# michalfratczak/habdec

Hardware: AMD Instinct MI355X
Metric: IQ Msamples/s (batched 2.048 MS/s streams) (higher is better)
Workload: dtype f32

## Files before the change

### habdec_amd/capi.py

```python
from __future__ import annotations

import ctypes as C
from pathlib import Path

import numpy as np

LIB_PATH = Path(__file__).resolve().parent / "libhabdec_amd.so"
_lib = None


class HabdecError(RuntimeError):
    pass


class hd_engine_config(C.Structure):
    _fields_ = [("device", C.c_int32), ("n_streams", C.c_uint32), ("max_chunk", C.c_uint32), ("sampling_rate", C.c_double),
                ("decimation", C.c_uint32), ("baud", C.c_double), ("rtty_bits", C.c_uint32), ("rtty_stops", C.c_float),
                ("lowpass_bw_hz", C.c_float), ("lowpass_trans", C.c_float), ("dc_remove", C.c_int32), ("lookup_mode", C.c_int32),
                ("enable_spectrum", C.c_int32), ("ungated", C.c_int32), ("keep_filtered", C.c_int32), ("pipeline", C.c_int32), ("arith", C.c_int32)]


class hd_afc_info(C.Structure):
    _fields_ = [("frequency_correction", C.c_double), ("shift_hz", C.c_double), ("noise_floor", C.c_double),
                ("noise_variance", C.c_double), ("peak_left", C.c_int32), ("peak_right", C.c_int32), ("spectra", C.c_uint64)]


class hd_timing(C.Structure):
    _fields_ = [("ms_total", C.c_double), ("ms_front", C.c_double), ("front_bytes", C.c_uint64), ("samples", C.c_uint64),
                ("host_enqueue_us", C.c_double), ("host_wait_us", C.c_double), ("host_text_us", C.c_double), ("timed_calls", C.c_uint64),
                ("path", C.c_uint32), ("step_variant", C.c_uint32), ("host_calls_in_place", C.c_uint64), ("lowpass_fft_calls", C.c_uint64)]


class hd_tune_info(C.Structure):
    _fields_ = [("offset_hz", C.c_double), ("step", C.c_uint32), ("phase", C.c_uint32), ("retunes", C.c_uint64), ("from_call", C.c_uint64),
                ("auto_afc", C.c_int32)]


class hd_front_tune_info(C.Structure):
    _fields_ = [("offset_hz", C.c_double), ("step", C.c_uint32), ("phase", C.c_uint32), ("from_call", C.c_uint64)]


SENTENCE_CB = C.CFUNCTYPE(None, C.c_void_p, C.c_uint32, C.c_char_p, C.c_char_p, C.c_char_p)
MATCH_CB = C.CFUNCTYPE(None, C.c_void_p, C.c_uint32, C.c_char_p, C.c_char_p, C.c_char_p, C.c_int)
CHARS_CB = C.CFUNCTYPE(None, C.c_void_p, C.c_uint32, C.POINTER(C.c_char), C.c_size_t)

# ... 27 lines not shown
    "hd_set_match_callback": (None, [_vp, MATCH_CB, _vp]),
    "hd_set_chars_callback": (None, [_vp, CHARS_CB, _vp]),
    "hd_process_host": (_int, [_vp, _vp, _sz, _vp, _u32]),
    "hd_process_device": (_int, [_vp, _vp, _sz, _vp, _u32]),
    "hd_flush": (_int, [_vp]),
    "hd_ingest_run": (_int, [_vp, _vp, C.c_uint64, C.POINTER(C.c_uint64)]),
    "hd_stream_rtty": (_sz, [_vp, _u32, C.c_char_p, _sz]),
    "hd_stream_last_sentence": (_sz, [_vp, _u32, C.c_char_p, _sz]),
    "hd_stream_take_sentences": (_sz, [_vp, _u32, C.c_char_p, _sz]),
    "hd_stream_take_matches": (_sz, [_vp, _u32, C.c_char_p, _sz]),
    "hd_stream_take_chars": (_sz, [_vp, _u32, C.c_char_p, _sz]),
    "hd_engine_sentences_ok": (C.c_uint64, [_vp]),
    "hd_stream_afc": (_int, [_vp, _u32, C.POINTER(hd_afc_info)]),
    "hd_stream_spectrum": (_sz, [_vp, _u32, _f32p, _sz]),
    "hd_stream_power": (_sz, [_vp, _u32, _f32p, _sz]),
    "hd_stream_demodulated": (_sz, [_vp, _u32, _f32p, _sz]),
    "hd_stream_decimated": (_sz, [_vp, _u32, _f32p, _sz]),
    "hd_stream_filtered": (_sz, [_vp, _u32, _f32p, _sz]),
    "hd_stream_bits": (_sz, [_vp, _u32, _u8p, _sz]),
    "hd_stream_flips": (_sz, [_vp, _u32, _u32p, _sz]),
    "hd_stream_fir_taps": (_sz, [_vp, _u32, _f32p, _sz]),
    "hd_stream_symbol_backlog": (_u32, [_vp, _u32]),
    "hd_stream_bits_total": (C.c_uint64, [_vp, _u32]),
    "hd_stream_flip_list_full": (C.c_uint64, [_vp, _u32]),
    "hd_stream_demod_checksum": (C.c_int, [_vp, _u32, C.POINTER(C.c_uint64), C.POINTER(C.c_uint32), C.POINTER(C.c_uint32)]),
    "hd_stream_demod_checksum_total": (C.c_int, [_vp, _u32, C.POINTER(C.c_uint64), C.POINTER(C.c_uint64), C.POINTER(C.c_uint64)]),
    "hd_min_chunk": (_u32, [_u32]),
    "hd_engine_timing": (_int, [_vp, C.POINTER(hd_timing)]),
    "hd_engine_set_timing": (None, [_vp, _int]),
}
# ... 67 lines not shown
```

### habdec_amd/csrc/dev_types.h

```cpp
#pragma once
#include <stdint.h>
#ifndef __HIPCC__
#ifndef __host__
#define __host__
#define __device__
#endif
#endif

namespace hd {

constexpr int kFftBins = 4096;
constexpr uint32_t kVentLimit = 30000;
constexpr uint32_t kFirBatch = 256;

struct StreamCall {
    uint32_t n_in;
    uint32_t n1;
    uint32_t n2;
    uint32_t zero_hist1;
    uint32_t zero_hist2;
    uint32_t pend_before;
    uint32_t fft_fill;
    uint32_t fft_take;
    uint32_t fft_run;
    uint32_t fir_m;
    uint32_t fir_taps;
    uint32_t fir_zero_hist;
    uint32_t pend_after;
    uint32_t dc_remove;
    uint32_t clear_pending;
    uint32_t fir_taps_prev;
};
__host__ __device__ inline uint32_t sc_taps_prev(const StreamCall& c) { return c.fir_taps_prev & 0xFFFFu; }
__host__ __device__ inline uint32_t sc_head_n(const StreamCall& c) { return (c.fir_taps_prev >> 16) & 0x3FFFu; }
__host__ __device__ inline bool sc_head_prev(const StreamCall& c) { return (c.fir_taps_prev >> 30) & 1u; }
__host__ __device__ inline bool sc_head_save(const StreamCall& c) { return (c.fir_taps_prev >> 31) & 1u; }
__host__ __device__ inline uint32_t sc_pack_taps_prev(uint32_t taps_prev, uint32_t head_n, bool head_prev, bool head_save)
{ return (taps_prev & 0xFFFFu) | ((head_n & 0x3FFFu) << 16) | ((head_prev ? 1u : 0u) << 30) | ((head_save ? 1u : 0u) << 31); }


struct SymbolParams {
    uint32_t spb;
    uint32_t R;
    uint32_t min_held;
    uint32_t float_abs;
    uint32_t reset;
};
// ... 33 lines not shown
```

### habdec_amd/csrc/engine.cpp

```cpp
#include <hip/hip_runtime.h>
#include <rocfft/rocfft.h>

#include <algorithm>
#include <atomic>
#include <chrono>
#include <cmath>
#include <cstdio>
#include <cstdlib>
#include <cstring>
#include <memory>
#include <condition_variable>
#include <mutex>
#include <thread>
#include <string>
#include <vector>

#include "../../include/habdec_amd.h"
#include "dev_types.h"
#include "host/afc_tracker.hpp"
#include "host/decim_plan.hpp"
#include "host/fir_design.hpp"
#include "host/iq_file_batch.hpp"
#include "host/text_stage.hpp"
#include "host/tune_host.hpp"
// ... 33 lines not shown
    hipError_t alloc(size_t count)
    {
        n = count;
        hipError_t e = hipHostMalloc(reinterpret_cast<void**>(&p), std::max<size_t>(count, 1) * sizeof(T), hipHostMallocMapped | hipHostMallocCoherent);
        if (e == hipSuccess) std::memset(p, 0, std::max<size_t>(count, 1) * sizeof(T));
        if (e == hipSuccess) e = hipHostGetDevicePointer(reinterpret_cast<void**>(&dev), p, 0);
        return e;
    }
    ~PinBuf() { if (p) (void)hipHostFree(p); }
};

struct SizeState {
    size_t stage_buf[2] = {0, 0};
    size_t pending = 0;
    size_t fft_fill = 0;
    size_t fir_buf = 0;
    uint32_t fir_T_run = 0;
    uint32_t head_n = 0;
    uint64_t head_call = ~0ull;
    bool head_aside = false;
    uint32_t tune_phase = 0;
    uint32_t front_phase = 0;
    uint32_t win_ub = 0, inflight_m = 0;
    uint32_t last_n2 = 0, last_pend_before = 0, last_m = 0;
    int last_buf = 0;
};

struct StreamHost {
    double baud = 300;
    float lp_bw = 1500, lp_trans = 0.025f;
    bool dc = false;
    hd::LowpassDesigner lp;
    bool taps_dirty = false;
    uint32_t tune_step = 0;
    uint32_t held = 0;
    bool sym_reset = true;
    hd::TextStage text;
    hd::AfcTracker afc;
    hd::SpectrumStats stats{};
    bool have_spectrum = false;
    uint64_t spectra = 0;
    uint32_t last_nbits = 0, last_nflips = 0;
    uint64_t flip_list_full = 0;
    uint64_t bits_total = 0;
    std::vector<uint32_t> last_words;
    uint32_t demod_ck[2] = {0, 0}, demod_ck_n = 0xFFFFFFFFu;
    uint64_t demod_ck_call = 0;
    uint64_t demod_ck_hash = 0xCBF29CE484222325ull;
    uint64_t demod_ck_calls = 0, demod_ck_unknown = 0;
    double tune_hz = 0;
    uint64_t tune_from = 0, retunes = 0;
    bool auto_afc = false;
    double afc_hold_s = 6.0, afc_min_hz = 100.0;
    uint64_t afc_elapsed = 0;
    double front_hz = 0;
// ... 9 lines not shown
    std::vector<hd::DecimStage> stages;
    uint32_t S = 0, D = 1;
    uint32_t n1_cap = 0, n2_cap = 0;
    uint32_t taps_cap = 0, fir_hist_cap = 0;
    size_t fbuf_stride = 0;
    uint32_t tail_cap = 0, backlog_cap = 0, slot_words = 0, flips_cap = 0, max_R = 0, min_R = 4;
    int bins_sep = 8;
    bool decode_enabled = true;
    bool fast = false;
    bool one_stream = false;
    bool no_tail = false;
    uint32_t tail_max_n2 = 2048;
    int last_route = -1;
    struct PendingTail { bool valid = false; hd::TailArgs ta{}; int slot = 0; int r2 = 0, t2 = 0; } pend;
    DevBuf<float2> fft_tw;
    bool no_claim = false;
    uint32_t step_run = 0;
    bool no_cu_step = false;
    uint32_t ring_run = 0;
    uint32_t ring_short_pct = 25;
    static constexpr uint32_t kS1Loaders = 2;
#ifndef HD_S1_SLOTS_BATCH
#define HD_S1_SLOTS_BATCH 4
#endif
    static constexpr uint32_t kS1Slots = HD_S1_SLOTS_BATCH;
    PinBuf<unsigned int> ring_gave_up;
    std::string fail_cause;
    bool device_failed = false;
    uint64_t step_launches = 0;
    DevBuf<unsigned int> step_ctr;
// ... 35 lines not shown
    DevBuf<uint32_t> demod_ck_acc;
    uint32_t head_cap = 0;
    DevBuf<hd::SymbolParams> d_sym;
    PinBuf<hd::SymbolParams> h_sym;
    static constexpr int kSlots = 4;
    struct CallSlot {
        DevBuf<hd::StreamCall> d_call;
        PinBuf<hd::StreamCall> h_call;
        PinBuf<uint32_t> h_slots;
        PinBuf<hd::SpectrumStatsDev> h_stats;
        PinBuf<uint2> h_tune;
        PinBuf<uint2> h_front;
        bool timed = false, timed_step = false;
        hipEvent_t ev_front = nullptr, ev_done = nullptr, ev_params = nullptr, ev_spec = nullptr, t0 = nullptr, t1 = nullptr, t2 = nullptr, t3 = nullptr;
        bool busy = false;
        uint32_t seq = 0;
        uint64_t total_in = 0;
        uint32_t r1 = 1;
        ~CallSlot() { for (hipEvent_t ev : {ev_front, ev_done, ev_params, ev_spec, t0, t1, t2, t3}) if (ev) (void)hipEventDestroy(ev); }
    } slot[kSlots];
    uint64_t calls = 0;
    uint64_t delivered = 0;
    int cur = 0;
    int hist_cur = 0;
    int carry_cur = 0;
    bool sym_dirty = true;

    std::vector<StreamHost> st;
    std::vector<SizeState> mirror, mirror_next;
    std::recursive_mutex mtx;
// ... 205 lines not shown
    HD_HIP(e->h_sym.alloc(S));
    for (auto& sl : e->slot) {
        HD_HIP(sl.d_call.alloc(S));
        HD_HIP(sl.h_call.alloc(S));
        HD_HIP(sl.h_slots.alloc((size_t)S * e->slot_words));
        HD_HIP(sl.h_tune.alloc(S));
        HD_HIP(sl.h_front.alloc(S));
    }
    {
        std::vector<float> tab(4 * hd::kTuneTable);
        hd::tune_tables(tab.data(), tab.data() + 2 * hd::kTuneTable);
        HD_HIP(e->tune_tab.alloc(tab.size()));
        HD_HIP(hipMemcpy(e->tune_tab.p, tab.data(), tab.size() * sizeof(float), hipMemcpyHostToDevice));
    }
    if (cfg->enable_spectrum) {
        HD_HIP(e->fft_in.alloc((size_t)S * hd::kFftBins));
        HD_HIP(e->spec.alloc((size_t)S * hd::kFftBins));
        HD_HIP(e->power.alloc((size_t)S * hd::kFftBins));
        for (auto& sl : e->slot) HD_HIP(sl.h_stats.alloc(S));
        {
            std::vector<float2> tw(hd::kFftBins);
            for (size_t m = 0; m < hd::kFftBins; ++m) {
                const double a = 2.0 * 3.14159265358979323846264338327950288 * (double)m / (double)hd::kFftBins;
                tw[m] = make_float2((float)std::cos(a), (float)-std::sin(a));
            }
            HD_HIP(e->fft_tw.alloc(hd::kFftBins));
            HD_HIP(hipMemcpy(e->fft_tw.p, tw.data(), tw.size() * sizeof(float2), hipMemcpyHostToDevice));
        }
    }
    if (e->fast && e->taps_cap >= hd_engine::kLpFftMinTaps && getenv("HD_NO_LP_FFT") == nullptr) {
        std::call_once(g_rocfft_once, [] { rocfft_setup(); });
// ... 65 lines not shown
    (void)hipDeviceSynchronize();
    delete e;
}

uint32_t hd_engine_streams(const hd_engine* e) { return e ? e->S : 0; }
uint32_t hd_engine_decimation(const hd_engine* e) { return e ? e->D : 0; }
double hd_engine_decimated_rate(const hd_engine* e) { return e ? e->fsd : 0; }
uint64_t hd_engine_sentences_ok(const hd_engine* e) { return e ? e->sentences_ok : 0; }
void hd_engine_set_timing(hd_engine* e, int on) { if (e) e->timing_every = on < 0 ? 0u : (uint32_t)on; }
int hd_engine_timing(hd_engine* e, hd_timing* out)
{
    if (!e || !out) return fail(HD_ERR_INVALID, "null argument");
    *out = e->last_timing;
    out->host_calls_in_place = e->host_calls_in_place;
    out->lowpass_fft_calls = e->lpf_calls;
    return HD_OK;
}

extern "C" int hd_debug_step_counters(hd_engine* e, unsigned int* out32)
{
    if (!e || !out32) return HD_ERR_INVALID;
    std::vector<unsigned int> h(2 * 16 * 32);
    if (hipDeviceSynchronize() != hipSuccess || hipMemcpy(h.data(), e->step_ctr.p, h.size() * 4, hipMemcpyDeviceToHost) != hipSuccess) return HD_ERR_DEVICE;
    for (int i = 0; i < 32; ++i) out32[i] = h[(size_t)i * 32];
    return HD_OK;
}

void hd_set_sentence_callback(hd_engine* e, hd_sentence_cb cb, void* user) { if (e) { e->sentence_cb = cb; e->sentence_user = user; } }
void hd_set_match_callback(hd_engine* e, hd_match_cb cb, void* user) { if (e) { e->match_cb = cb; e->match_user = user; } }
void hd_set_chars_callback(hd_engine* e, hd_chars_cb cb, void* user) { if (e) { e->chars_cb = cb; e->chars_user = user; } }
// ... 179 lines not shown
    }
    if (e->device_failed && rc == HD_OK)
        rc = fail(HD_ERR_DEVICE, e->fail_cause + ": the results of this and of every later call of this engine are unreliable -- destroy the engine");
    if (e->device_failed) {
        e->last_timing.host_wait_us = std::chrono::duration<double, std::micro>(w1 - w0).count();
        e->last_timing.host_text_us = 0;
        return rc;
    }
    for (uint32_t s = 0; s < e->S; ++s) {
        StreamHost& st = e->st[s];
        const hd::StreamCall& c = sl.h_call.p[s];
        if (c.fft_run) {
            std::memcpy(&st.stats, &sl.h_stats.p[s], sizeof(st.stats));
            st.have_spectrum = true;
            ++st.spectra;
        }
        const bool past_batch_gate = c.fir_m || c.clear_pending;
        if (past_batch_gate && e->cfg.enable_spectrum) st.afc.step(st.have_spectrum, st.stats, hd::kFftBins, e->fsd);
        st.afc_elapsed += c.n_in;
        if (st.auto_afc && (double)st.afc_elapsed >= st.afc_hold_s * e->fs && std::abs(st.afc.correction) > st.afc_min_hz) {
            const double corr = st.afc.correction;
            uint32_t d = 0;
            if (hd::tune_step(st.tune_hz + corr, e->fsd, &d)) {
                st.tune_hz += corr; st.tune_step = d; st.tune_from = e->calls;
                if (!d) e->mirror[s].tune_phase = 0;
                st.afc.reset(corr, hd::kFftBins, e->fsd);
                st.afc_elapsed = 0;
                ++st.retunes;
            }
        }
// ... 100 lines not shown
        const uint32_t n = n_per_stream ? n_per_stream[s] : n_uniform;
        c.n_in = n;
        c.n1 = n / p.R1;
        c.n2 = c.n1 / p.R2;
        if (n) {
            if (p.nst > 0) { const size_t want = (size_t)n + p.T1 + p.R1; if (nx.stage_buf[0] < want) { nx.stage_buf[0] = want; c.zero_hist1 = 1; } }
            if (p.nst > 1) { const size_t want = (size_t)c.n1 + p.T2 + p.R2; if (nx.stage_buf[1] < want) { nx.stage_buf[1] = want; c.zero_hist2 = 1; } }
        }
        c.dc_remove = st.dc && c.n2;
        sl.h_tune.p[s] = make_uint2(st.tune_step, nx.tune_phase);
        if (st.tune_step) { p.any_tune = true; nx.tune_phase += c.n2 * st.tune_step; }
        sl.h_front.p[s] = make_uint2(st.front_step, nx.front_phase);
        if (st.front_step | nx.front_phase) { p.any_front = true; nx.front_phase += n * st.front_step; }
        c.pend_before = (uint32_t)nx.pending;
        nx.pending += c.n2;
        c.fft_fill = (uint32_t)nx.fft_fill;
        if (e->cfg.enable_spectrum && n && nx.fft_fill < (size_t)hd::kFftBins && c.n2) {
            c.fft_take = (uint32_t)std::min<size_t>(hd::kFftBins - nx.fft_fill, c.n2);
            nx.fft_fill += c.fft_take;
        }
        if (e->cfg.enable_spectrum && n && nx.fft_fill >= (size_t)hd::kFftBins) { c.fft_run = 1; nx.fft_fill = 0; p.any_fft = true; }
        const bool past_batch_gate = n && nx.pending >= hd::kFirBatch;
        nx.last_m = 0;
        if (past_batch_gate && !e->decode_enabled) { c.clear_pending = 1; nx.pending = 0; }
        else if (past_batch_gate) {
            const uint32_t m = (uint32_t)(nx.pending - nx.pending % hd::kFirBatch);
            st.lp.batch = m;
            if (st.lp.design(cutoff_rel(e, st), st.lp_trans)) {
                st.taps_dirty = true;
                redesigned = true;
            }
            const uint32_t T = (uint32_t)st.lp.taps.size();
            if (!T) return fail(HD_ERR_UNSUPPORTED, "low-pass transition width leaves no taps (reference filters nothing then)");
            if (T > e->taps_cap) return fail(HD_ERR_CAPACITY, "low-pass tap count exceeds engine capacity");
            if (nx.fir_buf < (size_t)m + T) { nx.fir_buf = (size_t)m + T; c.fir_zero_hist = 1; }
            c.fir_m = m; c.fir_taps = T;
// ... 38 lines not shown
    r = CallRoute{};
    r.tail_lanes = S >= 2 * e->n_cus ? 64 : 256;
    const bool tail = p.nst == 2 && !p.any_dc && !e->no_tail && p.max_n2 <= e->tail_max_n2 &&
                      ((r.tail_lanes == 256 && p.max_n2 >= 512u && HDK(tail_layout, r.ta, r.tail_lanes, R2, T2, p.max_taps, e->max_R, e->min_R, e->tail_cap, p.max_pend, 64 * 1024, 4)) ||
                       HDK(tail_layout, r.ta, r.tail_lanes, R2, T2, p.max_taps, e->max_R, e->min_R, e->tail_cap, p.max_pend, 64 * 1024));
    const uint32_t step_lds = (p.R1 == 32 || p.R1 == 64) ? HDK(step_lds_bytes, (int)p.R1, (int)p.T1) : 0u;
    const bool step = tail && !p.any_front && e->cfg.pipeline && !e->one_stream && p.min_in == p.max_in && p.max_in && step_lds &&
                      HDK(tail_layout, r.ta_step, 64, R2, T2, p.max_taps, e->max_R, e->min_R, e->tail_cap, p.max_pend, step_lds);
    r.route = step ? Route::step : tail ? Route::tail : Route::separate;
    r.any_post = p.any_dc || (p.any_tune && !tail);
    r.lean = tail && !e->one_stream;
    r.free_front = !tail && p.nst == 2 && !e->one_stream;
    r.host_params = tail && !step && e->one_stream;
    r.dcall = r.host_params ? sl.h_call.dev : sl.d_call.p;
    r.feed = (e->cfg.enable_spectrum && !r.any_post) ? e->fft_in.p : nullptr;
    if (r.route != Route::separate || !e->cfg.enable_spectrum || r.any_post || !p.any_fft) return;
    for (uint32_t s = 0; s < S; ++s) {
        hd::StreamCall& c = sl.h_call.p[s];
        if (c.fft_run == 1 && c.fft_fill == 0 && c.fft_take == (uint32_t)hd::kFftBins) { c.fft_take = 0; c.fft_run = 2; }
    }
    r.spectrum_on_qc = !e->one_stream && p.nst != 0;
    for (uint32_t s = 0; s < S && r.spectrum_on_qc; ++s) r.spectrum_on_qc = sl.h_call.p[s].fft_run != 1u;
}

void fill_tail(const hd_engine* e, const hd_engine::CallSlot& sl, const CallPlan& p, const CallRoute& r, const CallBufs& b, hd::TailArgs& t)
{
    t.dec1 = b.d1; t.dec1_stride = e->n1_cap; t.hist2_in = e->hist2[b.hin].p; t.hist2_out = e->hist2[b.hout].p; t.taps2 = e->stage_taps[1].p;
    t.fbuf = b.fcur; t.fbuf_next = b.fnext; t.fbuf_stride = e->fbuf_stride; t.fir_hist_cap = e->fir_hist_cap;
    t.lp_taps = e->lp_taps.p; t.taps_stride = e->taps_cap; t.demod = e->demod.p; t.demod_stride = e->demod.n / e->S;
    t.filtered = e->cfg.keep_filtered ? e->filtered.p : nullptr; t.carry_in = e->carry[b.cin].p; t.carry_out = e->carry[b.cout].p;
    t.tune = p.any_tune ? sl.h_tune.dev : nullptr; t.tune_tab = e->tune_tab.p;
    t.call = r.dcall; t.fft_in = r.feed; t.head_buf = e->fir_head.p; t.fbuf_prev = b.fprev; t.head_cap = e->head_cap;
    t.n_streams = e->S;
    t.ring = e->tail.p; t.ring_cap = e->tail_cap; t.sym = e->d_symstate.p; t.flipmask = e->flipmask.p; t.wsum = e->weight.p;
    t.sp = e->d_sym.p; t.slots = sl.h_slots.dev; t.slot_words = e->slot_words; t.seq = sl.seq;
    t.flips_dbg = e->flips_cap ? e->flips_dbg.p : nullptr; t.flips_cap = e->flips_cap;
    t.fft_tw = r.feed ? e->fft_tw.p : nullptr;
    t.spec = e->spec.p; t.power = e->power.p; t.stats = sl.h_stats.dev; t.rate = e->fsd; t.bins_sep = e->bins_sep;
}

hd::StepClaim make_claim(const hd_engine* e, const CallPlan& p, uint32_t lin_wgs ,
                         uint32_t run_len_cu )
{
    hd::StepClaim claim{};
    const int R1 = (int)p.R1, T1 = (int)p.T1;
    const uint64_t S = e->S;
    const uint32_t ntiles = run_len_cu ? HDK(ring_tiles, R1, T1, p.max_in) : (p.max_n1 + 63) / 64, n_xcd = e->n_cus / 32u, run_len = run_len_cu ? run_len_cu : e->step_run >= 2 ? e->step_run : 4u;
    const uint64_t runs = S * ntiles / run_len;
    const bool shape_ok = run_len_cu ? (HDK(stage1_cu_supported, R1, T1) && p.max_in % 2048u == 0) : ((R1 == 32 || R1 == 64) && p.max_n1 % 64 == 0);
    if (!e->no_claim && (p.nst == 2 || (run_len_cu && p.nst == 1)) && shape_ok && p.min_in == p.max_in && p.max_in && !p.any_zero1 && n_xcd && e->n_cus % 32u == 0 && n_xcd <= 16 &&
        ntiles && (ntiles % run_len == 0 || (run_len_cu && R1 >= 32 && (S * ntiles) % run_len == 0)) && runs % n_xcd == 0 && S * ntiles < (1ull << 32) && (uint64_t)ntiles * S >= 4ull * lin_wgs) {
        claim.ctr = e->step_ctr.p + (size_t)(e->step_launches & 1u) * 16 * 32;
        claim.ctr_next = e->step_ctr.p + (size_t)((e->step_launches & 1u) ^ 1u) * 16 * 32;
// ... 108 lines not shown
            return fail(HD_ERR_INVALID, "no step kernel for this decimation plan");
        if (fb.ctr) ++e->step_launches;
    }
    if (sl.timed && !launched) HD_HIP(hipEventRecord(sl.t2, qa));
    if (ps && (!launched || sl.timed)) HD_HIP(hipEventRecord(ps->ev_done, qa));
    HD_HIP(hipGetLastError());
    return HD_OK;
}

void call_spectrum(hd_engine* e, hipStream_t q, hd_engine::CallSlot& sl, const CallPlan& p, const CallRoute& r)
{
    if (!(e->cfg.enable_spectrum && p.max_n2)) return;
    const float2* fcur = e->fbuf[e->cur].p;
    if (r.any_post || p.nst == 0) HDK(launch_fft_feed, q, e->S, fcur, e->fbuf_stride, e->fft_in.p, r.dcall, e->fir_hist_cap);
    if (!p.any_fft) return;
    hd::launch_spectrum_wave(q, e->S, e->fft_in.p, e->fft_tw.p, e->spec.p, e->power.p, sl.h_stats.dev, r.dcall, e->fsd, e->bins_sep, sl.seq, fcur, e->fbuf_stride, e->fir_hist_cap);
}

int enqueue_front(hd_engine* e, hd_engine::CallSlot& sl, const CallPlan& p, const CallRoute& r, const float2* iq, size_t stride)
{
    const uint32_t S = e->S, R1 = p.R1, T1 = p.T1;
    const bool tail = r.route == Route::tail;
    hipStream_t qa = e->qa;
    const CallBufs b = call_bufs(e);
    if (p.nst == 0) {
        if (sl.timed) HD_HIP(hipEventRecord(sl.t1, qa));
        HDK(launch_passthrough, qa, S, p.max_in, iq, stride, b.fcur, e->fbuf_stride, r.dcall, e->fir_hist_cap);
        if (sl.timed) HD_HIP(hipEventRecord(sl.t2, qa));
    } else {
        const bool single = p.nst == 1;
        float2* out1 = single ? b.fcur : b.d1;
// ... 342 lines not shown
size_t hd_stream_take_chars(hd_engine* e, uint32_t s, char* buf, size_t cap)
{ if (check_stream(e, s)) return 0; std::lock_guard<std::recursive_mutex> l(e->mtx); return take_out(e->st[s].text.char_log, buf, cap); }

int hd_stream_afc(hd_engine* e, uint32_t s, hd_afc_info* out)
{
    if (int r = check_stream(e, s)) return r;
    if (!out) return fail(HD_ERR_INVALID, "null argument");
    std::lock_guard<std::recursive_mutex> l(e->mtx);
    const StreamHost& st = e->st[s];
    out->frequency_correction = st.afc.correction; out->shift_hz = st.afc.shift_hz;
    out->noise_floor = st.afc.noise_floor; out->noise_variance = st.afc.noise_sigma;
    out->peak_left = st.afc.gui_left; out->peak_right = st.afc.gui_right; out->spectra = st.spectra;
    return HD_OK;
}

static size_t fetch(hd_engine* e, const void* dev, size_t count, size_t elem, void* host, size_t cap)
{
    if (e->in_callback) { fail(HD_ERR_INVALID, "data getters cannot be called from a sentence / character callback (text getters can)"); return 0; }
    (void)flush_locked(e);
    const size_t n = std::min(count, cap);
    if (!n || !host) return count;
    if (hipSetDevice(e->cfg.device) != hipSuccess) return 0;
    if (hipMemcpy(host, dev, n * elem, hipMemcpyDeviceToHost) != hipSuccess) return 0;
    return count;
}

size_t hd_stream_spectrum(hd_engine* e, uint32_t s, float* iq, size_t cap)
{
    if (check_stream(e, s)) return 0;
    std::lock_guard<std::recursive_mutex> l(e->mtx);
    if (!e->cfg.enable_spectrum || !e->st[s].have_spectrum) return 0;
    return fetch(e, e->spec.p + (size_t)s * hd::kFftBins, hd::kFftBins, sizeof(float2), iq, cap);
}
size_t hd_stream_power(hd_engine* e, uint32_t s, float* p, size_t cap)
{
    if (check_stream(e, s)) return 0;
    std::lock_guard<std::recursive_mutex> l(e->mtx);
    if (!e->cfg.enable_spectrum || !e->st[s].have_spectrum) return 0;
    return fetch(e, e->power.p + (size_t)s * hd::kFftBins, hd::kFftBins, sizeof(float), p, cap);
}
size_t hd_stream_demodulated(hd_engine* e, uint32_t s, float* v, size_t cap)
{
    if (check_stream(e, s)) return 0;
    std::lock_guard<std::recursive_mutex> l(e->mtx);
    return fetch(e, e->demod.p + (size_t)s * (e->demod.n / e->S), e->mirror[s].last_m, sizeof(float), v, cap);
}
size_t hd_stream_decimated(hd_engine* e, uint32_t s, float* iq, size_t cap)
{
    if (check_stream(e, s)) return 0;
    std::lock_guard<std::recursive_mutex> l(e->mtx);
    const SizeState& sz = e->mirror[s];
    const float2* src = e->fbuf[sz.last_buf].p + (size_t)s * e->fbuf_stride + e->fir_hist_cap + sz.last_pend_before;
    return fetch(e, src, sz.last_n2, sizeof(float2), iq, cap);
}
// ... 72 lines not shown
```

### habdec_amd/csrc/kernels/launch.h

```cpp
#pragma once
#include <hip/hip_runtime.h>
#include <stddef.h>
#include <stdint.h>

#include "../dev_types.h"

namespace hd {

struct DemodCarry {
    float re, im;
    uint32_t primed;
    uint32_t _pad;
};

struct StepClaim {
    unsigned int* ctr = nullptr;
    unsigned int* ctr_next = nullptr;
    uint32_t n_xcd = 0, runs_per_xcd = 0, run_len = 0;
    uint32_t short_from = 0xFFFFFFFFu, tiles_per_xcd = 0;
};

struct TailArgs {
    const float2* dec1; size_t dec1_stride;
    const float2* hist2_in; float2* hist2_out; const float* taps2;
// ... 7 lines not shown
    uint32_t* slots; uint32_t slot_words; uint32_t* flips_dbg; uint32_t flips_cap;
    uint32_t seq;
    const float2* fft_tw; float2* spec; float* power; SpectrumStatsDev* stats; double rate; int bins_sep;
    uint32_t pend_max, f_off, v_off, ws_off, words_off, tp_off, h2_off, flips_off, fl_cap, strips_off, dyn_off, lds_bytes;
    uint32_t op;
    const uint2* tune; const float* tune_tab;
};

constexpr uint32_t kStepLdsBytes = 20480;

void launch_spectrum_wave(hipStream_t st, uint32_t n_streams, const float2* fft_in, const float2* tw4096, float2* spec, float* power,
                          SpectrumStatsDev* stats, const StreamCall* call, double rate, int bins_sep,
                          uint32_t seq ,
                          const float2* chunk = nullptr ,
                          size_t chunk_stride = 0, uint32_t fir_hist_cap = 0);

namespace exact {
#include "launch_decls.inc"
}
namespace fast {
#include "launch_decls.inc"
}

}
```

### habdec_amd/csrc/kernels/spectrum_wave.h

```cpp
#pragma once
#include <hip/hip_runtime.h>

#include "launch.h"
#include "sym_common.h"

namespace hd {

namespace specwave {

__device__ static constexpr float kW64[2][32] = {
#include "fft64_tw.inc"
};

constexpr int xpos(int k) { return 8 * (k & 7) + (k >> 3); }

__device__ __forceinline__ void fft8(f32x2 (&v)[8])
{
    constexpr float r = 0.70710678118654752440f;
    const f32x2 a0 = v[0] + v[4], a1 = v[0] - v[4], a2 = v[2] + v[6], a3 = v[2] - v[6];
    const f32x2 a4 = v[1] + v[5], a5 = v[1] - v[5], a6 = v[3] + v[7], a7 = v[3] - v[7];
    const f32x2 a3r = (f32x2){a3.y, -a3.x}, a7r = (f32x2){a7.y, -a7.x};
    const f32x2 b0 = a0 + a2, b2 = a0 - a2, b1 = a1 + a3r, b3 = a1 - a3r;
    const f32x2 b4 = a4 + a6, b6 = a4 - a6, b5 = a5 + a7r, b7 = a5 - a7r;
    const f32x2 t5 = (f32x2){(b5.x + b5.y) * r, (b5.y - b5.x) * r};
// ... 103 lines not shown
    for (int k1 = 0; k1 < 64; ++k1) plane[k1 * 65 + l] = a[specwave::xpos(k1)].y;
    __builtin_amdgcn_s_waitcnt(0xC07F);
    __builtin_amdgcn_wave_barrier();
#pragma unroll
    for (int n2 = 0; n2 < 64; ++n2) a[n2].y = plane[l * 65 + n2];
    specwave::pin64(a);
    specwave::fft64(a);
    specwave::pin64(a);
    float2* so = spec + (size_t)s * kFftBins;
    float* po = power + (size_t)s * kFftBins;
    int mybad = 0;
    double lsum = 0.0;
#define HD_SW_P(j_) a[specwave::xpos(((j_) + 32) & 63)].x
    float2* sg = so;
    float* pg = po;
#pragma unroll
    for (int j = 0; j < 64; ++j) {
        if ((j & 7) == 0) {
            __builtin_amdgcn_sched_barrier(0);
            sg = so + 64 * j; pg = po + 64 * j;
            asm volatile("" : "+s"(sg), "+s"(pg));
        }
        const int k2 = (j + 32) & 63;
        const f32x2 v = a[specwave::xpos(k2)];
        sg[l + 64 * (j & 7)] = make_float2(v.x, v.y);
        float q = (v.x * v.x + v.y * v.y) / (float)kFftBins;
        q = q * q;
        q = (float)((double)q / rate);
        q = 10.0f * log10f(q);
        if (v.x != v.x || v.y != v.y || isinf(v.x) || isinf(v.y) || q != q || isinf(q)) mybad = 1;
        HD_SW_P(j) = q;
        pg[l + 64 * (j & 7)] = q;
        lsum += (double)q;
    }
    const bool bad = __builtin_amdgcn_ballot_w64(mybad != 0) != 0ull;
    const double mean = specwave::wave_sum(lsum) / (double)kFftBins;
    double lvar = 0.0;
    float bv = -__builtin_huge_valf();
    int bi = kFftBins;
#pragma unroll
    for (int j = 0; j < 64; ++j) {
        const float pj = HD_SW_P(j);
        const double d = (double)pj - mean;
        lvar += d * d;
        if (pj > bv) { bv = pj; bi = (int)l + 64 * j; }
    }
    const double sigma = sqrt(specwave::wave_sum(lvar) / (double)kFftBins);
    specwave::wave_argmax(bv, bi);
    const int p1 = bi;
    const float p1v = bv;
    const int lo = max(p1 - 2 * bins_sep, 0), hi = min(p1 + 2 * bins_sep, (int)kFftBins);
    const float floor0 = __shfl(HD_SW_P(0), 0, 64);
    float cv = -__builtin_huge_valf();
    int ci = kFftBins;
#pragma unroll
    for (int j = 0; j < 64; ++j) {
        const int i = (int)l + 64 * j;
        const float pj = HD_SW_P(j);
        if (i >= lo && i < hi && pj > floor0 && abs(i - p1) > bins_sep / 2 && pj > cv) { cv = pj; ci = i; }
    }
    specwave::wave_argmax(cv, ci);
    if (l == 0) {
        int pa = p1, pb = 0;
        float av = p1v, bvv = floor0;
        if (ci < (int)kFftBins) { pb = ci; bvv = cv; }
        if (pb < pa) { const int ti = pa; pa = pb; pb = ti; const float tv = av; av = bvv; bvv = tv; }
        SpectrumStatsDev o;
        o.valid = bad ? 0 : 1;
        o.peak1 = pa; o.peak2 = pb; o.power1 = av; o.power2 = bvv; o.seq = 0u;
        o.mean = mean; o.sigma = sigma;
        stats[s] = o;
        asm volatile("s_waitcnt vmcnt(0)" ::: "memory");
        __hip_atomic_store(&stats[s].seq, seq, __ATOMIC_RELAXED, __HIP_MEMORY_SCOPE_SYSTEM);
    }
#undef HD_SW_P
}

// ... 2 lines not shown
```

### habdec_amd/csrc/kernels/spectrum_wave.hip

```cpp
#include <hip/hip_runtime.h>

#include "spectrum_wave.h"

namespace hd {

__global__ __launch_bounds__(64) __attribute__((amdgpu_waves_per_eu(2, 2))) void k_spectrum_wave(const float2* __restrict__ fft_in, const float2* __restrict__ tw4096, float2* __restrict__ spec,
                                                        float* __restrict__ power, SpectrumStatsDev* __restrict__ stats,
                                                        const StreamCall* __restrict__ call, double rate, int bins_sep, const uint32_t seq,
                                                        const float2* __restrict__ chunk, const size_t chunk_stride, const uint32_t fir_hist_cap)
{
    __shared__ float plane[64 * 65];
    const uint32_t s = blockIdx.x;
    const uint32_t run = call[s].fft_run;
    if (!run) return;
    const float2* x = run == 2u ? chunk + (size_t)s * chunk_stride + fir_hist_cap + call[s].pend_before : fft_in + (size_t)s * kFftBins;
    spectrum_wave_body(x, tw4096, spec, power, stats, s, rate, bins_sep, plane, seq);
}

void launch_spectrum_wave(hipStream_t st, uint32_t n_streams, const float2* fft_in, const float2* tw4096, float2* spec, float* power,
                          SpectrumStatsDev* stats, const StreamCall* call, double rate, int bins_sep, uint32_t seq, const float2* chunk, size_t chunk_stride, uint32_t fir_hist_cap)
{
    hipLaunchKernelGGL(k_spectrum_wave, dim3(n_streams), dim3(64), 0, st, fft_in, tw4096, spec, power, stats, call, rate, bins_sep, seq, chunk, chunk_stride, fir_hist_cap);
}

}
```

### habdec_amd/csrc/kernels/tail_body.h

```cpp
#pragma once
#include <hip/hip_runtime.h>

#include "arith.h"
#include "exact_math.h"
#include "launch.h"
#include "sym_common.h"
#include "spectrum_wave.h"
#include "tune.h"

namespace hd {
namespace HD_ARITH_NS {

constexpr uint32_t kTailHdrBytes = 64;
constexpr uint32_t kTailStrip = 512;

typedef float f32x4 __attribute__((ext_vector_type(4)));
typedef const float __attribute__((address_space(4)))* cfloat_ptr;
__device__ __forceinline__ cfloat_ptr as_const(const float* p) { return (cfloat_ptr)(uintptr_t)p; }

#define HD_TB_TAP4(A_, B_, C_, D_, k_)                                                        \
    {                                                                                         \
        HD_FIR_ARITH                                                                          \
        const f32x2 p0_ = (A_) * (k_), p1_ = (B_) * (k_), p2_ = (C_) * (k_), p3_ = (D_) * (k_); \
        a0 = a0 + p0_; a1 = a1 + p1_; a2 = a2 + p2_; a3 = a3 + p3_;                           \
// ... 866 lines not shown
        if constexpr (NT == 64) {
            if (tid == 0) { hdr->demod_ck[0] = ck0; hdr->demod_ck[1] = ck1; hdr->demod_n = m; }
        } else {
            tb_sync<NT>();
            if (tid == 0) { sh[5] = 0; sh[6] = 0; }
            tb_sync<NT>();
            if (lane == 0) { atomicAdd(&sh[5], ck0); atomicAdd(&sh[6], ck1); }
            tb_sync<NT>();
            if (tid == 0) { hdr->demod_ck[0] = sh[5]; hdr->demod_ck[1] = sh[6]; hdr->demod_n = m; }
        }
    }
    if (a.fft_tw && c.fft_run) {
        __threadfence_block();
        tb_sync<NT>();
        if (wave == 0)
            spectrum_wave_body(a.fft_in + (size_t)s * kFftBins, a.fft_tw, a.spec, a.power, a.stats, s, a.rate, a.bins_sep, reinterpret_cast<float*>(lds + kTailHdrBytes), a.seq);
    }
    asm volatile("s_waitcnt vmcnt(0)" ::: "memory");
#ifdef HD_RING_FAULT
    if (tid == 0 && g_tail_fault_armed && atomicCAS(&g_tail_fault_fired, 0u, 1u) == 0u) return;
#endif
    if (tid == 0) __hip_atomic_store(&hdr->seq, a.seq, __ATOMIC_RELAXED, __HIP_MEMORY_SCOPE_SYSTEM);
    TSTAMP_WRITE();
}

}
}
```

### habdec_amd/engine.py

```python
from __future__ import annotations

import ctypes as C
from dataclasses import dataclass

import numpy as np

from . import capi
from .capi import HabdecError, check, lib


@dataclass
class EngineConfig:
    n_streams: int = 1
    max_chunk: int = 65536
    sampling_rate: float = 2.048e6
    decimation: int = 64
    baud: float = 300.0
    rtty_bits: int = 8
    rtty_stops: float = 2.0
    lowpass_bw_hz: float = 1500.0
    lowpass_trans: float = 0.025
    dc_remove: bool = False
    lookup_mode: int = 1
    enable_spectrum: bool = True
# ... 114 lines not shown
        a = capi.hd_afc_info()
        check(self.L.hd_stream_afc(self.h, s, C.byref(a)))
        return {"correction": a.frequency_correction, "shift_hz": a.shift_hz, "noise_floor": a.noise_floor,
                "noise_var": a.noise_variance, "peak_l": a.peak_left, "peak_r": a.peak_right, "spectra": a.spectra}

    def _arr(self, fn, s, cplx, cap):
        buf = np.zeros(cap * (2 if cplx else 1), np.float32)
        n = fn(self.h, s, buf, cap)
        if n > cap:
            return self._arr(fn, s, cplx, n)
        out = buf[: n * (2 if cplx else 1)]
        return out.view(np.complex64) if cplx else out

    def spectrum(self, s=0): return self._arr(self.L.hd_stream_spectrum, s, True, 4096)
    def power(self, s=0): return self._arr(self.L.hd_stream_power, s, False, 4096)
    def demodulated(self, s=0): return self._arr(self.L.hd_stream_demodulated, s, False, 1 << 15)
    def decimated(self, s=0): return self._arr(self.L.hd_stream_decimated, s, True, 1 << 16)
    def filtered(self, s=0): return self._arr(self.L.hd_stream_filtered, s, True, 1 << 15)
    def fir_taps(self, s=0): return self._arr(self.L.hd_stream_fir_taps, s, False, 8192)

    def bits(self, s=0) -> np.ndarray:
        cap = 1 << 16
        buf = np.zeros(cap, np.uint8)
        n = self.L.hd_stream_bits(self.h, s, buf, cap)
        return buf[:n].copy()

    def flips(self, s=0) -> np.ndarray:
        buf = np.zeros(4096, np.uint32)
        n = self.L.hd_stream_flips(self.h, s, buf, 4096)
        return buf[:n].copy()
# ... 6 lines not shown
    def demod_checksum(self, s=0):
        ci, n, ck = C.c_uint64(0), C.c_uint32(0), (C.c_uint32 * 2)()
        check(self.L.hd_stream_demod_checksum(self.h, s, C.byref(ci), C.byref(n), ck))
        return int(ci.value), (None if n.value == 0xFFFFFFFF else int(n.value)), int(ck[0]), int(ck[1])

    def demod_checksum_total(self, s=0):
        n, u, h = C.c_uint64(0), C.c_uint64(0), C.c_uint64(0)
        check(self.L.hd_stream_demod_checksum_total(self.h, s, C.byref(n), C.byref(u), C.byref(h)))
        return int(n.value), int(u.value), int(h.value)

    def timing(self) -> dict:
        t = capi.hd_timing()
        check(self.L.hd_engine_timing(self.h, C.byref(t)))
        return {"ms_total": t.ms_total, "ms_front": t.ms_front, "front_bytes": t.front_bytes, "samples": t.samples,
                "host_enqueue_us": t.host_enqueue_us, "host_wait_us": t.host_wait_us, "host_text_us": t.host_text_us,
                "timed_calls": t.timed_calls, "path": t.path, "step_variant": t.step_variant, "host_calls_in_place": t.host_calls_in_place, "lowpass_fft_calls": t.lowpass_fft_calls}

    def set_timing(self, every: int):
        self.L.hd_engine_set_timing(self.h, every)


class IqFiles:

    def __init__(self, paths, chunk: int, granule: int, loop: bool = False, realtime_rate: float = 0.0):
        import ctypes as C
        self.L = lib()
        arr = (C.c_char_p * len(paths))(*[str(p).encode() for p in paths])
        self.h = self.L.hd_host_iqfiles_open(arr, len(paths), int(loop), chunk, granule, realtime_rate)
        if not self.h:
            raise HabdecError("hd_host_iqfiles_open failed (missing file, chunk < granule, ...)")
        self.S, self.chunk = len(paths), chunk
# ... 23 lines not shown
```

### include/habdec_amd.h

```cpp
#ifndef HABDEC_AMD_H
#define HABDEC_AMD_H

#include <stddef.h>
#include <stdint.h>

#ifdef __cplusplus
extern "C" {
#endif

#define HD_OK 0
#define HD_ERR_INVALID (-1)
#define HD_ERR_DEVICE (-2)
#define HD_ERR_UNSUPPORTED (-3)
#define HD_ERR_CAPACITY (-4)

#define HD_FFT_BINS 4096

typedef struct hd_engine hd_engine;

typedef struct hd_engine_config {
    int32_t  device;
    uint32_t n_streams;
    uint32_t max_chunk;
    double   sampling_rate;
// ... 68 lines not shown
size_t hd_stream_rtty(hd_engine* e, uint32_t stream, char* buf, size_t cap);
size_t hd_stream_last_sentence(hd_engine* e, uint32_t stream, char* buf, size_t cap);
size_t hd_stream_take_sentences(hd_engine* e, uint32_t stream, char* buf, size_t cap);
size_t hd_stream_take_matches(hd_engine* e, uint32_t stream, char* buf, size_t cap);
size_t hd_stream_take_chars(hd_engine* e, uint32_t stream, char* buf, size_t cap);
uint64_t hd_engine_sentences_ok(const hd_engine* e);

typedef struct hd_afc_info {
    double frequency_correction, shift_hz, noise_floor, noise_variance;
    int32_t peak_left, peak_right;
    uint64_t spectra;
} hd_afc_info;
int    hd_stream_afc(hd_engine* e, uint32_t stream, hd_afc_info* out);
size_t hd_stream_spectrum(hd_engine* e, uint32_t stream, float* iq, size_t cap_complex);
size_t hd_stream_power(hd_engine* e, uint32_t stream, float* p, size_t cap);
size_t hd_stream_demodulated(hd_engine* e, uint32_t stream, float* v, size_t cap);

size_t hd_stream_decimated(hd_engine* e, uint32_t stream, float* iq, size_t cap_complex);
size_t hd_stream_filtered(hd_engine* e, uint32_t stream, float* iq, size_t cap_complex);
size_t hd_stream_bits(hd_engine* e, uint32_t stream, uint8_t* bits, size_t cap);
size_t hd_stream_flips(hd_engine* e, uint32_t stream, uint32_t* flips, size_t cap);
size_t hd_stream_fir_taps(hd_engine* e, uint32_t stream, float* taps, size_t cap);
uint32_t hd_stream_symbol_backlog(hd_engine* e, uint32_t stream);
int hd_stream_demod_checksum(hd_engine* e, uint32_t stream, uint64_t* call_index, uint32_t* n, uint32_t ck[2]);
int hd_stream_demod_checksum_total(hd_engine* e, uint32_t stream, uint64_t* calls, uint64_t* calls_without, uint64_t* hash);
uint64_t hd_stream_bits_total(hd_engine* e, uint32_t stream);
uint64_t hd_stream_flip_list_full(hd_engine* e, uint32_t stream);

typedef struct hd_timing {
    double ms_total;
    double ms_front;
    uint64_t front_bytes;
    uint64_t samples;
    double host_enqueue_us;
    double host_wait_us;
    double host_text_us;
    uint64_t timed_calls;
    uint32_t path;
    uint32_t step_variant;
    uint64_t host_calls_in_place;
    uint64_t lowpass_fft_calls;
} hd_timing;
int hd_engine_timing(hd_engine* e, hd_timing* out);
void hd_engine_set_timing(hd_engine* e, int every);

#ifdef __cplusplus
}
#endif
#endif
```

Measured before the change: 505,000.

## Defer spectrum and power stores to on-demand refresh in batch mode

In pipeline (batch) mode the per-call spectrum kernel no longer writes the full 4096-bin complex spectrum and power arrays. It only computes the stats the AFC needs and keeps the FFT input in a double-buffered row. A new refresh kernel recomputes spectrum and power for stale streams when a getter or the new refresh API asks for them. This removes large per-call global stores, at the cost of twice the fft_in memory, a packed row index in StreamCall::fft_fill, and a synchronous recompute on read.

```diff
diff --git a/habdec_amd/capi.py b/habdec_amd/capi.py
--- a/habdec_amd/capi.py
+++ b/habdec_amd/capi.py
@@ -28,7 +28,8 @@
 class hd_timing(C.Structure):
     _fields_ = [("ms_total", C.c_double), ("ms_front", C.c_double), ("front_bytes", C.c_uint64), ("samples", C.c_uint64),
                 ("host_enqueue_us", C.c_double), ("host_wait_us", C.c_double), ("host_text_us", C.c_double), ("timed_calls", C.c_uint64),
-                ("path", C.c_uint32), ("step_variant", C.c_uint32), ("host_calls_in_place", C.c_uint64), ("lowpass_fft_calls", C.c_uint64)]
+                ("path", C.c_uint32), ("step_variant", C.c_uint32), ("host_calls_in_place", C.c_uint64), ("lowpass_fft_calls", C.c_uint64),
+                ("spectrum_refresh_launches", C.c_uint64)]
 
 
 class hd_tune_info(C.Structure):
@@ -86,6 +87,7 @@
     "hd_stream_afc": (_int, [_vp, _u32, C.POINTER(hd_afc_info)]),
     "hd_stream_spectrum": (_sz, [_vp, _u32, _f32p, _sz]),
     "hd_stream_power": (_sz, [_vp, _u32, _f32p, _sz]),
+    "hd_streams_refresh_spectra": (_int, [_vp, _vp, _u32]),
     "hd_stream_demodulated": (_sz, [_vp, _u32, _f32p, _sz]),
     "hd_stream_decimated": (_sz, [_vp, _u32, _f32p, _sz]),
     "hd_stream_filtered": (_sz, [_vp, _u32, _f32p, _sz]),
diff --git a/habdec_amd/csrc/dev_types.h b/habdec_amd/csrc/dev_types.h
--- a/habdec_amd/csrc/dev_types.h
+++ b/habdec_amd/csrc/dev_types.h
@@ -31,6 +31,9 @@
     uint32_t clear_pending;
     uint32_t fir_taps_prev;
 };
+__host__ __device__ inline uint32_t sc_fft_fill(const StreamCall& c) { return c.fft_fill & 0xFFFu; }
+__host__ __device__ inline uint32_t sc_fft_row(const StreamCall& c) { return c.fft_fill >> 12; }
+__host__ __device__ inline uint32_t sc_pack_fft_fill(uint32_t fill, uint32_t row) { return (fill & 0xFFFu) | (row << 12); }
 __host__ __device__ inline uint32_t sc_taps_prev(const StreamCall& c) { return c.fir_taps_prev & 0xFFFFu; }
 __host__ __device__ inline uint32_t sc_head_n(const StreamCall& c) { return (c.fir_taps_prev >> 16) & 0x3FFFu; }
 __host__ __device__ inline bool sc_head_prev(const StreamCall& c) { return (c.fir_taps_prev >> 30) & 1u; }
diff --git a/habdec_amd/csrc/engine.cpp b/habdec_amd/csrc/engine.cpp
--- a/habdec_amd/csrc/engine.cpp
+++ b/habdec_amd/csrc/engine.cpp
@@ -71,6 +71,7 @@
     size_t stage_buf[2] = {0, 0};
     size_t pending = 0;
     size_t fft_fill = 0;
+    uint32_t fft_par = 0;
     size_t fir_buf = 0;
     uint32_t fir_T_run = 0;
     uint32_t head_n = 0;
@@ -96,6 +97,8 @@
     hd::AfcTracker afc;
     hd::SpectrumStats stats{};
     bool have_spectrum = false;
+    bool spec_stale = false;
+    uint32_t spec_row = 0;
     uint64_t spectra = 0;
     uint32_t last_nbits = 0, last_nflips = 0;
     uint64_t flip_list_full = 0;
@@ -135,6 +138,9 @@
     int last_route = -1;
     struct PendingTail { bool valid = false; hd::TailArgs ta{}; int slot = 0; int r2 = 0, t2 = 0; } pend;
     DevBuf<float2> fft_tw;
+    bool spectra_on_demand = false;
+    PinBuf<uint2> refresh_list;
+    uint64_t refresh_launches = 0;
     bool no_claim = false;
     uint32_t step_run = 0;
     bool no_cu_step = false;
@@ -200,6 +206,7 @@
         bool timed = false, timed_step = false;
         hipEvent_t ev_front = nullptr, ev_done = nullptr, ev_params = nullptr, ev_spec = nullptr, t0 = nullptr, t1 = nullptr, t2 = nullptr, t3 = nullptr;
         bool busy = false;
+        bool spec_stored = true;
         uint32_t seq = 0;
         uint64_t total_in = 0;
         uint32_t r1 = 1;
@@ -435,7 +442,10 @@
         HD_HIP(hipMemcpy(e->tune_tab.p, tab.data(), tab.size() * sizeof(float), hipMemcpyHostToDevice));
     }
     if (cfg->enable_spectrum) {
-        HD_HIP(e->fft_in.alloc((size_t)S * hd::kFftBins));
+        e->spectra_on_demand = cfg->pipeline != 0;
+        if (e->spectra_on_demand && S >= (1u << 19)) return fail(HD_ERR_CAPACITY, "a batch-mode engine with spectra takes fewer than 2^19 streams (StreamCall::fft_fill carries the collection row)");
+        HD_HIP(e->fft_in.alloc((size_t)S * hd::kFftBins * (e->spectra_on_demand ? 2u : 1u)));
+        if (e->spectra_on_demand) HD_HIP(e->refresh_list.alloc(S));
         HD_HIP(e->spec.alloc((size_t)S * hd::kFftBins));
         HD_HIP(e->power.alloc((size_t)S * hd::kFftBins));
         for (auto& sl : e->slot) HD_HIP(sl.h_stats.alloc(S));
@@ -531,6 +541,7 @@
     *out = e->last_timing;
     out->host_calls_in_place = e->host_calls_in_place;
     out->lowpass_fft_calls = e->lpf_calls;
+    out->spectrum_refresh_launches = e->refresh_launches;
     return HD_OK;
 }
 
@@ -740,6 +751,8 @@
             std::memcpy(&st.stats, &sl.h_stats.p[s], sizeof(st.stats));
             st.have_spectrum = true;
             ++st.spectra;
+            st.spec_stale = !sl.spec_stored;
+            st.spec_row = s + hd::sc_fft_row(c);
         }
         const bool past_batch_gate = c.fir_m || c.clear_pending;
         if (past_batch_gate && e->cfg.enable_spectrum) st.afc.step(st.have_spectrum, st.stats, hd::kFftBins, e->fsd);
@@ -870,12 +883,15 @@
         if (st.front_step | nx.front_phase) { p.any_front = true; nx.front_phase += n * st.front_step; }
         c.pend_before = (uint32_t)nx.pending;
         nx.pending += c.n2;
-        c.fft_fill = (uint32_t)nx.fft_fill;
+        c.fft_fill = hd::sc_pack_fft_fill((uint32_t)nx.fft_fill, nx.fft_par ? e->S : 0u);
         if (e->cfg.enable_spectrum && n && nx.fft_fill < (size_t)hd::kFftBins && c.n2) {
             c.fft_take = (uint32_t)std::min<size_t>(hd::kFftBins - nx.fft_fill, c.n2);
             nx.fft_fill += c.fft_take;
         }
-        if (e->cfg.enable_spectrum && n && nx.fft_fill >= (size_t)hd::kFftBins) { c.fft_run = 1; nx.fft_fill = 0; p.any_fft = true; }
+        if (e->cfg.enable_spectrum && n && nx.fft_fill >= (size_t)hd::kFftBins) {
+            c.fft_run = 1; nx.fft_fill = 0; p.any_fft = true;
+            if (e->spectra_on_demand) nx.fft_par ^= 1u;
+        }
         const bool past_batch_gate = n && nx.pending >= hd::kFirBatch;
         nx.last_m = 0;
         if (past_batch_gate && !e->decode_enabled) { c.clear_pending = 1; nx.pending = 0; }
@@ -944,10 +960,11 @@
     r.host_params = tail && !step && e->one_stream;
     r.dcall = r.host_params ? sl.h_call.dev : sl.d_call.p;
     r.feed = (e->cfg.enable_spectrum && !r.any_post) ? e->fft_in.p : nullptr;
+    sl.spec_stored = !e->spectra_on_demand;
     if (r.route != Route::separate || !e->cfg.enable_spectrum || r.any_post || !p.any_fft) return;
     for (uint32_t s = 0; s < S; ++s) {
         hd::StreamCall& c = sl.h_call.p[s];
-        if (c.fft_run == 1 && c.fft_fill == 0 && c.fft_take == (uint32_t)hd::kFftBins) { c.fft_take = 0; c.fft_run = 2; }
+        if (c.fft_run == 1 && hd::sc_fft_fill(c) == 0 && c.fft_take == (uint32_t)hd::kFftBins) { c.fft_take = 0; c.fft_run = 2; sl.spec_stored = true; }
     }
     r.spectrum_on_qc = !e->one_stream && p.nst != 0;
     for (uint32_t s = 0; s < S && r.spectrum_on_qc; ++s) r.spectrum_on_qc = sl.h_call.p[s].fft_run != 1u;
@@ -966,7 +983,7 @@
     t.sp = e->d_sym.p; t.slots = sl.h_slots.dev; t.slot_words = e->slot_words; t.seq = sl.seq;
     t.flips_dbg = e->flips_cap ? e->flips_dbg.p : nullptr; t.flips_cap = e->flips_cap;
     t.fft_tw = r.feed ? e->fft_tw.p : nullptr;
-    t.spec = e->spec.p; t.power = e->power.p; t.stats = sl.h_stats.dev; t.rate = e->fsd; t.bins_sep = e->bins_sep;
+    t.spec = sl.spec_stored ? e->spec.p : nullptr; t.power = sl.spec_stored ? e->power.p : nullptr; t.stats = sl.h_stats.dev; t.rate = e->fsd; t.bins_sep = e->bins_sep;
 }
 
 hd::StepClaim make_claim(const hd_engine* e, const CallPlan& p, uint32_t lin_wgs ,
@@ -1105,7 +1122,7 @@
     const float2* fcur = e->fbuf[e->cur].p;
     if (r.any_post || p.nst == 0) HDK(launch_fft_feed, q, e->S, fcur, e->fbuf_stride, e->fft_in.p, r.dcall, e->fir_hist_cap);
     if (!p.any_fft) return;
-    hd::launch_spectrum_wave(q, e->S, e->fft_in.p, e->fft_tw.p, e->spec.p, e->power.p, sl.h_stats.dev, r.dcall, e->fsd, e->bins_sep, sl.seq, fcur, e->fbuf_stride, e->fir_hist_cap);
+    hd::launch_spectrum_wave(q, e->S, e->fft_in.p, e->fft_tw.p, sl.spec_stored ? e->spec.p : nullptr, sl.spec_stored ? e->power.p : nullptr, sl.h_stats.dev, r.dcall, e->fsd, e->bins_sep, sl.seq, fcur, e->fbuf_stride, e->fir_hist_cap);
 }
 
 int enqueue_front(hd_engine* e, hd_engine::CallSlot& sl, const CallPlan& p, const CallRoute& r, const float2* iq, size_t stride)
@@ -1478,6 +1495,33 @@
     return HD_OK;
 }
 
+static int refresh_spectra(hd_engine* e, const uint32_t* streams, uint32_t n)
+{
+    if (!e->spectra_on_demand) return 0;
+    if (e->in_callback) return fail(HD_ERR_INVALID, "data getters cannot be called from a sentence / character callback (text getters can)");
+    if (hipSetDevice(e->cfg.device) != hipSuccess) return fail(HD_ERR_DEVICE, "hipSetDevice failed");
+    if (const int rc = flush_locked(e)) return rc;
+    if (e->device_failed) return fail(HD_ERR_DEVICE, "this engine is in its failed state (" + e->fail_cause + ") -- destroy the engine");
+    uint32_t k = 0;
+    const uint32_t cnt = streams ? n : e->S;
+    for (uint32_t i = 0; i < cnt; ++i) {
+        const uint32_t s = streams ? streams[i] : i;
+        if (s >= e->S) return fail(HD_ERR_INVALID, "stream index out of range");
+        StreamHost& st = e->st[s];
+        if (!st.have_spectrum || !st.spec_stale) continue;
+        st.spec_stale = false;
+        e->refresh_list.p[k++] = make_uint2(s, st.spec_row);
+    }
+    if (!k) return 0;
+    hd::launch_spectrum_refresh(e->qa, k, e->fft_in.p, e->fft_tw.p, e->spec.p, e->power.p, e->refresh_list.dev, e->fsd, e->bins_sep);
+    ++e->refresh_launches;
+    if (hipGetLastError() != hipSuccess || hipStreamSynchronize(e->qa) != hipSuccess) {
+        for (uint32_t i = 0; i < k; ++i) e->st[e->refresh_list.p[i].x].spec_stale = true;
+        return fail(HD_ERR_DEVICE, "the spectrum refresh launch failed");
+    }
+    return (int)k;
+}
+
 static size_t fetch(hd_engine* e, const void* dev, size_t count, size_t elem, void* host, size_t cap)
 {
     if (e->in_callback) { fail(HD_ERR_INVALID, "data getters cannot be called from a sentence / character callback (text getters can)"); return 0; }
@@ -1493,15 +1537,25 @@
 {
     if (check_stream(e, s)) return 0;
     std::lock_guard<std::recursive_mutex> l(e->mtx);
-    if (!e->cfg.enable_spectrum || !e->st[s].have_spectrum) return 0;
+    if (!e->cfg.enable_spectrum) return 0;
+    if (e->spectra_on_demand && refresh_spectra(e, &s, 1) < 0) return 0;
+    if (!e->st[s].have_spectrum) return 0;
     return fetch(e, e->spec.p + (size_t)s * hd::kFftBins, hd::kFftBins, sizeof(float2), iq, cap);
 }
 size_t hd_stream_power(hd_engine* e, uint32_t s, float* p, size_t cap)
 {
     if (check_stream(e, s)) return 0;
     std::lock_guard<std::recursive_mutex> l(e->mtx);
-    if (!e->cfg.enable_spectrum || !e->st[s].have_spectrum) return 0;
+    if (!e->cfg.enable_spectrum) return 0;
+    if (e->spectra_on_demand && refresh_spectra(e, &s, 1) < 0) return 0;
+    if (!e->st[s].have_spectrum) return 0;
     return fetch(e, e->power.p + (size_t)s * hd::kFftBins, hd::kFftBins, sizeof(float), p, cap);
+}
+int hd_streams_refresh_spectra(hd_engine* e, const uint32_t* streams, uint32_t n)
+{
+    if (!e) return fail(HD_ERR_INVALID, "null engine");
+    std::lock_guard<std::recursive_mutex> l(e->mtx);
+    return refresh_spectra(e, streams, n);
 }
 size_t hd_stream_demodulated(hd_engine* e, uint32_t s, float* v, size_t cap)
 {
diff --git a/habdec_amd/csrc/kernels/launch.h b/habdec_amd/csrc/kernels/launch.h
--- a/habdec_amd/csrc/kernels/launch.h
+++ b/habdec_amd/csrc/kernels/launch.h
@@ -45,6 +45,7 @@
                           uint32_t seq ,
                           const float2* chunk = nullptr ,
                           size_t chunk_stride = 0, uint32_t fir_hist_cap = 0);
+void launch_spectrum_refresh(hipStream_t st, uint32_t n, const float2* fft_in, const float2* tw4096, float2* spec, float* power, const uint2* list, double rate, int bins_sep);
 
 namespace exact {
 #include "launch_decls.inc"
diff --git a/habdec_amd/csrc/kernels/spectrum_wave.h b/habdec_amd/csrc/kernels/spectrum_wave.h
--- a/habdec_amd/csrc/kernels/spectrum_wave.h
+++ b/habdec_amd/csrc/kernels/spectrum_wave.h
@@ -141,6 +141,7 @@
 #define HD_SW_P(j_) a[specwave::xpos(((j_) + 32) & 63)].x
     float2* sg = so;
     float* pg = po;
+    const bool st_spec = spec != nullptr, st_power = power != nullptr;
 #pragma unroll
     for (int j = 0; j < 64; ++j) {
         if ((j & 7) == 0) {
@@ -150,14 +151,14 @@
         }
         const int k2 = (j + 32) & 63;
         const f32x2 v = a[specwave::xpos(k2)];
-        sg[l + 64 * (j & 7)] = make_float2(v.x, v.y);
+        if (st_spec) sg[l + 64 * (j & 7)] = make_float2(v.x, v.y);
         float q = (v.x * v.x + v.y * v.y) / (float)kFftBins;
         q = q * q;
         q = (float)((double)q / rate);
         q = 10.0f * log10f(q);
         if (v.x != v.x || v.y != v.y || isinf(v.x) || isinf(v.y) || q != q || isinf(q)) mybad = 1;
         HD_SW_P(j) = q;
-        pg[l + 64 * (j & 7)] = q;
+        if (st_power) pg[l + 64 * (j & 7)] = q;
         lsum += (double)q;
     }
     const bool bad = __builtin_amdgcn_ballot_w64(mybad != 0) != 0ull;
@@ -187,7 +188,7 @@
         if (i >= lo && i < hi && pj > floor0 && abs(i - p1) > bins_sep / 2 && pj > cv) { cv = pj; ci = i; }
     }
     specwave::wave_argmax(cv, ci);
-    if (l == 0) {
+    if (l == 0 && stats) {
         int pa = p1, pb = 0;
         float av = p1v, bvv = floor0;
         if (ci < (int)kFftBins) { pb = ci; bvv = cv; }
diff --git a/habdec_amd/csrc/kernels/spectrum_wave.hip b/habdec_amd/csrc/kernels/spectrum_wave.hip
--- a/habdec_amd/csrc/kernels/spectrum_wave.hip
+++ b/habdec_amd/csrc/kernels/spectrum_wave.hip
@@ -13,8 +13,16 @@
     const uint32_t s = blockIdx.x;
     const uint32_t run = call[s].fft_run;
     if (!run) return;
-    const float2* x = run == 2u ? chunk + (size_t)s * chunk_stride + fir_hist_cap + call[s].pend_before : fft_in + (size_t)s * kFftBins;
+    const float2* x = run == 2u ? chunk + (size_t)s * chunk_stride + fir_hist_cap + call[s].pend_before : fft_in + ((size_t)s + sc_fft_row(call[s])) * kFftBins;
     spectrum_wave_body(x, tw4096, spec, power, stats, s, rate, bins_sep, plane, seq);
+}
+
+__global__ __launch_bounds__(64) __attribute__((amdgpu_waves_per_eu(2, 2))) void k_spectrum_refresh(const float2* __restrict__ fft_in, const float2* __restrict__ tw4096, float2* __restrict__ spec,
+                                                           float* __restrict__ power, const uint2* __restrict__ list, double rate, int bins_sep)
+{
+    __shared__ float plane[64 * 65];
+    const uint2 e = list[blockIdx.x];
+    spectrum_wave_body(fft_in + (size_t)e.y * kFftBins, tw4096, spec, power, nullptr, e.x, rate, bins_sep, plane, 0u);
 }
 
 void launch_spectrum_wave(hipStream_t st, uint32_t n_streams, const float2* fft_in, const float2* tw4096, float2* spec, float* power,
@@ -23,4 +31,9 @@
     hipLaunchKernelGGL(k_spectrum_wave, dim3(n_streams), dim3(64), 0, st, fft_in, tw4096, spec, power, stats, call, rate, bins_sep, seq, chunk, chunk_stride, fir_hist_cap);
 }
 
+void launch_spectrum_refresh(hipStream_t st, uint32_t n, const float2* fft_in, const float2* tw4096, float2* spec, float* power, const uint2* list, double rate, int bins_sep)
+{
+    if (n) hipLaunchKernelGGL(k_spectrum_refresh, dim3(n), dim3(64), 0, st, fft_in, tw4096, spec, power, list, rate, bins_sep);
 }
+
+}
diff --git a/habdec_amd/csrc/kernels/tail_body.h b/habdec_amd/csrc/kernels/tail_body.h
--- a/habdec_amd/csrc/kernels/tail_body.h
+++ b/habdec_amd/csrc/kernels/tail_body.h
@@ -904,7 +904,7 @@
         __threadfence_block();
         tb_sync<NT>();
         if (wave == 0)
-            spectrum_wave_body(a.fft_in + (size_t)s * kFftBins, a.fft_tw, a.spec, a.power, a.stats, s, a.rate, a.bins_sep, reinterpret_cast<float*>(lds + kTailHdrBytes), a.seq);
+            spectrum_wave_body(a.fft_in + ((size_t)s + sc_fft_row(c)) * kFftBins, a.fft_tw, a.spec, a.power, a.stats, s, a.rate, a.bins_sep, reinterpret_cast<float*>(lds + kTailHdrBytes), a.seq);
     }
     asm volatile("s_waitcnt vmcnt(0)" ::: "memory");
 #ifdef HD_RING_FAULT
diff --git a/habdec_amd/engine.py b/habdec_amd/engine.py
--- a/habdec_amd/engine.py
+++ b/habdec_amd/engine.py
@@ -152,6 +152,16 @@
 
     def spectrum(self, s=0): return self._arr(self.L.hd_stream_spectrum, s, True, 4096)
     def power(self, s=0): return self._arr(self.L.hd_stream_power, s, False, 4096)
+    def refresh_spectra(self, streams=None) -> int:
+        if streams is None:
+            n = self.L.hd_streams_refresh_spectra(self.h, None, 0)
+        else:
+            a = np.ascontiguousarray(streams, np.uint32)
+            n = self.L.hd_streams_refresh_spectra(self.h, a.ctypes.data, a.size)
+        if n < 0:
+            check(n)
+        return n
+
     def demodulated(self, s=0): return self._arr(self.L.hd_stream_demodulated, s, False, 1 << 15)
     def decimated(self, s=0): return self._arr(self.L.hd_stream_decimated, s, True, 1 << 16)
     def filtered(self, s=0): return self._arr(self.L.hd_stream_filtered, s, True, 1 << 15)
@@ -188,7 +198,8 @@
         check(self.L.hd_engine_timing(self.h, C.byref(t)))
         return {"ms_total": t.ms_total, "ms_front": t.ms_front, "front_bytes": t.front_bytes, "samples": t.samples,
                 "host_enqueue_us": t.host_enqueue_us, "host_wait_us": t.host_wait_us, "host_text_us": t.host_text_us,
-                "timed_calls": t.timed_calls, "path": t.path, "step_variant": t.step_variant, "host_calls_in_place": t.host_calls_in_place, "lowpass_fft_calls": t.lowpass_fft_calls}
+                "timed_calls": t.timed_calls, "path": t.path, "step_variant": t.step_variant, "host_calls_in_place": t.host_calls_in_place, "lowpass_fft_calls": t.lowpass_fft_calls,
+                "spectrum_refresh_launches": t.spectrum_refresh_launches}
 
     def set_timing(self, every: int):
         self.L.hd_engine_set_timing(self.h, every)
diff --git a/include/habdec_amd.h b/include/habdec_amd.h
--- a/include/habdec_amd.h
+++ b/include/habdec_amd.h
@@ -106,6 +106,7 @@
 int    hd_stream_afc(hd_engine* e, uint32_t stream, hd_afc_info* out);
 size_t hd_stream_spectrum(hd_engine* e, uint32_t stream, float* iq, size_t cap_complex);
 size_t hd_stream_power(hd_engine* e, uint32_t stream, float* p, size_t cap);
+int hd_streams_refresh_spectra(hd_engine* e, const uint32_t* streams, uint32_t n);
 size_t hd_stream_demodulated(hd_engine* e, uint32_t stream, float* v, size_t cap);
 
 size_t hd_stream_decimated(hd_engine* e, uint32_t stream, float* iq, size_t cap_complex);
@@ -132,6 +133,7 @@
     uint32_t step_variant;
     uint64_t host_calls_in_place;
     uint64_t lowpass_fft_calls;
+    uint64_t spectrum_refresh_launches;
 } hd_timing;
 int hd_engine_timing(hd_engine* e, hd_timing* out);
 void hd_engine_set_timing(hd_engine* e, int every);
```

Result: no change. 514,500 (median of 6 runs) (+1.9%).
